# akofke/fountain

Measured on AMD Instinct MI355X. Metric: Mrays/s (primary+secondary) at fixed spp, higher is better.
Workload: dtype f32; 1 GPU; config 5 scene: 2309 baked copies of rounded_cube = 10002588 triangles (19979703 BVH nodes, depth 29), 4096x4096 film, PathIntegrator(max_depth 5, rr 1.0), 1024^2 env-map light; one step = 16 spp over the whole film; tiles=65536, tiles_per_gpu=65536, pipeline=wavefront, sampler=indexed xoshiro256+, per_gpu_workload=copies=2309,res=4096,spp_per_gpu=16

## Files before the change

fountain_amd/csrc/ftn_trace4.hip:

```cpp
#include "ftn_wf_common.h"

namespace ftn {

enum : uint32_t { T4_IDLE = 0, T4_NODE = 1, T4_LEAF = 2 };
#define T4_NONE 0xffffffffu

typedef float t4_f2 __attribute__((ext_vector_type(2)));
__device__ inline bool slab4(float4 a, float4 b, V3 o, V3 inv, float t_max, float* t0o, float* t1o) {
    const float k = 1.0f + 2.0f * gamma_n(3);
    const t4_f2 px = {a.x, a.y}, py = {a.z, a.w}, pz = {b.x, b.y};
    const t4_f2 tx = (px - (t4_f2){o.x, o.x}) * (t4_f2){inv.x, inv.x};
    const t4_f2 ty = (py - (t4_f2){o.y, o.y}) * (t4_f2){inv.y, inv.y};
    const t4_f2 tz = (pz - (t4_f2){o.z, o.z}) * (t4_f2){inv.z, inv.z};
    const float far_k = fmin_(fmin_(fmax_(tx.x, tx.y), fmax_(ty.x, ty.y)), fmax_(tz.x, tz.y)) * k;
    const float t0 = fmax_(fmax_(fmax_(0.0f, fmin_(tx.x, tx.y)), fmin_(ty.x, ty.y)), fmin_(tz.x, tz.y));
    const float t1 = fmin_(t_max, far_k);
    *t0o = t0; *t1o = t1;
    return !(t0 > t1);
}

struct WaveQueue {
    uint32_t chunk_next, chunk_end, slice, slices_done, chunk; bool exhausted;
};
__device__ inline void wq_init(WaveQueue& q, uint32_t count, uint32_t chunk_max) {
// ... 110 lines not shown
    const float4 q0 = rec[0], q1 = rec[1], q2 = rec[2], q3 = rec[3], q4 = rec[4], q5 = rec[5], q6 = rec[6], q7 = rec[7];
    float ta, tb, tc, td, x1;
    const bool ha = slab4(q0, q1, R.o, R.inv, R.t_max, &ta, &x1), hb = slab4(q2, q3, R.o, R.inv, R.t_max, &tb, &x1);
    const bool hc = slab4(q4, q5, R.o, R.inv, R.t_max, &tc, &x1), hd = slab4(q6, q7, R.o, R.inv, R.t_max, &td, &x1);
    const uint32_t ea = ha ? __float_as_uint(q1.z) : T4_NONE, eb = hb ? __float_as_uint(q3.z) : T4_NONE, ec = hc ? __float_as_uint(q5.z) : T4_NONE, ed = hd ? __float_as_uint(q7.z) : T4_NONE;
    t4_visit<CHECK>(St, L, R.t_max, ea, eb, ec, ed, ta, tb, tc, td, __float_as_uint(q1.w) & R.neg24);
}

template <bool CHECK>
__device__ __forceinline__ void t4q_record_step(const DScene& S, T4Stack<uint2>& St, T4Lane& L, V3 o, V3 inv, float t_max, uint32_t neg24) {
    const uint4* rec = reinterpret_cast<const uint4*>(reinterpret_cast<const char*>(S.quad64) + L.cur);
    const uint4 r0 = rec[0], r1 = rec[1], r2 = rec[2], r3 = rec[3];
    const float k2 = 1.0f + 4.0f * gamma_n(3);
    const T8Axis X = t8_axis(__uint_as_float(r0.x), r0.w & 0xffu, o.x, inv.x, r1.x, r1.x, r1.y, r1.y);
    const T8Axis Y = t8_axis(__uint_as_float(r0.y), (r0.w >> 8) & 0xffu, o.y, inv.y, r1.z, r1.z, r1.w, r1.w);
    const T8Axis Z = t8_axis(__uint_as_float(r0.z), (r0.w >> 16) & 0xffu, o.z, inv.z, r2.x, r2.x, r2.y, r2.y);
    float ta, a1, tb, b1, tc, c1, td, d1;
    T8_CHILD(0, ta, a1) T8_CHILD(1, tb, b1) T8_CHILD(2, tc, c1) T8_CHILD(3, td, d1)
    const uint32_t ea = !(ta > a1) ? r2.z : T4_NONE, eb = !(tb > b1) ? r2.w : T4_NONE, ec = !(tc > c1) ? r3.x : T4_NONE, ed = !(td > d1) ? r3.y : T4_NONE;
    t4_visit<CHECK>(St, L, t_max, ea, eb, ec, ed, ta, tb, tc, td, r3.z & neg24);
}

enum : uint32_t { T4_LEAF_IN = 3 };
template <bool COUNT, bool SPHERES, int BURST, bool Q64 = false>
__global__ void __launch_bounds__(256, (SPHERES ? 1 : (Q64 ? T4Q_WAVES : 5))) k_wf_trace4(DScene S, WfBuffers W, const uint32_t* __restrict__ queue, const uint32_t* count_ptr, uint32_t* head, DevStats* stats,
                                                   uint32_t refill, uint32_t leaf_batch, uint32_t chunk_max, uint32_t lds_entries, uint2* __restrict__ spill, uint32_t spill_levels) {
    T4Stack<uint2> St;
    extern __shared__ uint2 lds_stack2[];
    St.base = lds_stack2 + threadIdx.x;
    St.lim = St.base + 256u * lds_entries; St.sp = St.base; St.spill = spill; St.spill_levels = spill_levels;
    St.n_lanes = (size_t)gridDim.x * 256u; St.gl = (size_t)blockIdx.x * 256u + threadIdx.x;
    const bool st_tiny = lds_entries < 3u;
    uint2* const st_soft = st_tiny ? St.base : St.lim - 3 * 256;
    const uint32_t count = *count_ptr;
    const uint32_t lane = lane_id();
    unsigned long long n_rec = 0, n_prim = 0;
    unsigned long long occ[7] = {0, 0, 0, 0, 0, 0, 0};
    T4Lane L; L.mode = T4_IDLE; L.cur = 0; L.lp = 0; L.finish = false;
    WaveQueue Q; wq_init(Q, count, chunk_max);
    uint32_t rid = 0;
    RaySetup R; R.o = V3(0.0f, 0.0f, 0.0f); R.inv = R.o; R.dorig = R.o; R.t_max = 0.0f; R.neg24 = 0; R.kz = 0; R.sx = R.sy = R.sz = 0.0f;
    int hprim = -1; float hb0 = 0.0f, hb1 = 0.0f, hb2 = 0.0f; bool found = false;
    const float4 rlo = make_float4(S.root_lo[0], S.root_lo[1], S.root_lo[2], 0.0f), rhi = make_float4(S.root_hi[0], S.root_hi[1], S.root_hi[2], 0.0f);
    for (;;) {
        const unsigned long long idle = __ballot(L.mode == T4_IDLE);
        if (!Q.exhausted && (uint32_t)__popcll(idle) >= refill) {
            const uint32_t need = (uint32_t)__popcll(idle);
            if (wq_refill(Q, count, head, lane)) {
                if (W.drain_sig && lane == 0 && atomicAdd(&W.counters[CTR(WFC_DRY_WAVES)], 1u) + 1u == W.drain_at)
                    __hip_atomic_store(W.drain_sig, W.drain_seq, __ATOMIC_RELAXED, __HIP_MEMORY_SCOPE_SYSTEM);
            }
            const uint32_t avail = Q.chunk_end - Q.chunk_next;
            const uint32_t rank = (uint32_t)__popcll(idle & ((1ull << lane) - 1ull));
            bool hand_back = false; uint32_t q_entry = 0;
            if (COUNT) { occ[5]++; occ[6] += need < avail ? need : avail; }
            if (L.mode == T4_IDLE && rank < avail) {
                float4 a, b;
                q_entry = queue[Q.chunk_next + rank];
                load_queued_ray<false>(W, q_entry, &a, &b, &rid);
                ray_setup<SPHERES>(R, a, b);
                St.sp = St.base; L.cur = 0; found = false; hprim = -1; hb0 = 0.0f; hb1 = 0.0f; hb2 = 0.0f;
                if (ray_is_exceptional(R.o.x, R.o.y, R.o.z, R.inv.x, R.inv.y, R.inv.z) || (Q64 && ray_out_of_range8(R.o.x, R.o.y, R.o.z, R.inv.x, R.inv.y, R.inv.z)))
                    hand_back = true;
                else if (S.n_nodes == 0 || !slab_test(rlo, rhi, R.o, R.inv, R.t_max)) { W.hit[rid] = make_float4(FTN_INF, 0.0f, 0.0f, 0.0f); W.hit_prim[rid] = -1; }
                else if (S.root_is_leaf) { L.lp = 0; L.mode = T4_LEAF; }
                else L.mode = T4_NODE;
            }
            if (__ballot(hand_back) != 0) wave_push(hand_back, q_entry, W.q_exc_closest, &W.counters[CTR(WFC_EXC_CLOSEST)]);
            Q.chunk_next += (need < avail ? need : avail);
        }
        const unsigned long long m_node = __ballot(L.mode == T4_NODE), m_leaf = __ballot(L.mode >= T4_LEAF);
        if ((m_node | m_leaf) == 0) { if (Q.exhausted) break; else continue; }
        L.finish = false;
        if (COUNT) occ[0]++;
        if (m_node != 0 && (uint32_t)__popcll(m_leaf) < leaf_batch) {
#pragma unroll
            for (int burst = 0; burst < BURST; burst++) {
                const bool on = L.mode == T4_NODE && !L.finish;
                if (COUNT && on) n_rec++;
                if (COUNT) { const unsigned long long m_on = __ballot(on); if (m_on) { occ[1]++; occ[2] += (unsigned long long)__popcll(m_on); } }
                if (__builtin_expect(__ballot(on && (st_tiny || St.sp > st_soft)) == 0, 1)) {
                    if (on) { if (Q64) t4q_record_step<false>(S, St, L, R.o, R.inv, R.t_max, R.neg24); else t4_record_step<false>(S, R, St, L); }
// ... 306 lines not shown
        const uint32_t wg_q = knob_wg_closest ? knob_wg_closest : (uint32_t)T4Q_WAVES, budget_q = ((158u * 1024u) / wg_q) & ~1023u;
        const uint32_t bound_q = S.quad64_stack_bound ? S.quad64_stack_bound : 1u;
        uint32_t eq = knob_entries_closest ? knob_entries_closest : budget_q / (256u * 8u);
        p.entries_q64 = eq < bound_q ? eq : bound_q;
        if (p.entries_q64 == 0) p.entries_q64 = 1;
        p.spill_q64 = bound_q - p.entries_q64;
        p.lds_q64 = (size_t)p.entries_q64 * 256u * 8u;
        p.grid_q64 = (unsigned)n_cu * per_cu(p.lds_q64, wg_q);
        p.q64_ok = true;
    }
    if (S.oct && S.n_octs) {
        const uint32_t wg_8 = knob_wg_oct ? knob_wg_oct : 5u, budget_8 = ((158u * 1024u) / wg_8) & ~1023u, bound8 = S.oct_stack_bound ? S.oct_stack_bound : 1u;
        const uint32_t e8 = knob_entries_oct ? knob_entries_oct : budget_8 / (256u * 4u);
        p.entries_oct = e8 < bound8 ? e8 : bound8;
        p.spill_oct = bound8 - p.entries_oct;
        p.lds_oct = (size_t)p.entries_oct * 256u * 4u;
        p.grid_oct = (unsigned)n_cu * per_cu(p.lds_oct, wg_8);
        p.oct_ok = true;
    }
    return p;
}

void launch_trace4(int kind, bool count, bool spheres, unsigned grid, size_t lds, uint32_t lds_entries, void* spill, hipStream_t stream, const DScene& S, const WfBuffers& W,
                   const uint32_t* queue, const uint32_t* count_ptr, uint32_t* head, DevStats* stats, uint32_t refill, uint32_t leaf_batch, uint32_t chunk, uint32_t burst, uint32_t any_policy, uint32_t spill_levels) {
    const bool any = kind == T4K_ANY || kind == T4K_ANY_OCT;
#define FTN_T4(K, SPILL_T, ...) hipLaunchKernelGGL((K<__VA_ARGS__>), dim3(grid), dim3(256), lds, stream, S, W, queue, count_ptr, head, stats, refill, leaf_batch, chunk, lds_entries, (SPILL_T)spill, spill_levels)
    if (kind == T4K_CLOSEST_Q64) {
        if (count) FTN_T4(k_wf_trace4, uint2*, true, false, 2, true);
        else if (burst <= 1) FTN_T4(k_wf_trace4, uint2*, false, false, 1, true); else if (burst == 2) FTN_T4(k_wf_trace4, uint2*, false, false, 2, true);
        else if (burst == 3) FTN_T4(k_wf_trace4, uint2*, false, false, 3, true); else FTN_T4(k_wf_trace4, uint2*, false, false, 4, true);
    } else if (kind == T4K_ANY_OCT) {
#define FTN_T8(C, B) do { if (any_policy == 0) FTN_T4(k_wf_trace8_any, uint32_t*, C, B, 0); else FTN_T4(k_wf_trace8_any, uint32_t*, C, B, 1); } while (0)
        if (count) FTN_T8(true, 2);
        else if (burst <= 1) FTN_T8(false, 1); else if (burst == 2) FTN_T8(false, 2); else FTN_T8(false, 3);
#undef FTN_T8
    } else if (any) {
#define FTN_T4A(C, Sp, B) do { if (any_policy == 0) FTN_T4(k_wf_trace4_any, uint32_t*, C, Sp, B, 0); else FTN_T4(k_wf_trace4_any, uint32_t*, C, Sp, B, 1); } while (0)
        if (count) { if (spheres) FTN_T4A(true, true, 2); else FTN_T4A(true, false, 2); }
        else if (spheres) { if (burst <= 2) FTN_T4A(false, true, 2); else FTN_T4A(false, true, 4); }
        else { if (burst <= 1) FTN_T4A(false, false, 1); else if (burst == 2) FTN_T4A(false, false, 2); else if (burst == 3) FTN_T4A(false, false, 3); else FTN_T4A(false, false, 4); }
#undef FTN_T4A
    } else {
        if (count) { if (spheres) FTN_T4(k_wf_trace4, uint2*, true, true, 2); else FTN_T4(k_wf_trace4, uint2*, true, false, 2); }
        else if (spheres) { if (burst <= 2) FTN_T4(k_wf_trace4, uint2*, false, true, 2); else FTN_T4(k_wf_trace4, uint2*, false, true, 4); }
        else { if (burst <= 1) FTN_T4(k_wf_trace4, uint2*, false, false, 1); else if (burst == 2) FTN_T4(k_wf_trace4, uint2*, false, false, 2); else if (burst == 3) FTN_T4(k_wf_trace4, uint2*, false, false, 3); else FTN_T4(k_wf_trace4, uint2*, false, false, 4); }
    }
#undef FTN_T4
}

}
// ... 1 lines not shown
```

fountain_amd/csrc/ftn_wavefront.hip:

```cpp
#include "ftn_wf_internal.h"
#include "ftn_wf_path.h"
#include "ftn_texture.h"
#include <algorithm>
#include <cstdlib>
#include <cstring>
#include <vector>

namespace ftn {

__global__ void __launch_bounds__(256) k_wf_generate(RenderParams P, WfBuffers W, int write_state) {
    const uint32_t i = blockIdx.x * 256u + threadIdx.x;
    if (i >= W.n_paths) return;
    const uint32_t slot = i / W.samples, s = i % W.samples;
    const DTile tile = P.tiles[slot >> 8];
    const int px = tile.x0 + (int)(slot & 15u), py = tile.y0 + (int)((slot >> 4) & 15u);
    if (px < tile.x1 && py < tile.y1) {
        Rng rng; rng.seed(indexed_key(P.seed, px, py, W.first_sample + s));
        V2 j = rng.next2();
        V2 p_film((float)px + j.x, (float)py + j.y);
        V2 p_lens = rng.next2();
        float time_u = rng.next();
        DRay ray = camera_ray(P.C, p_film, p_lens, time_u);
        W.ray[2 * (size_t)(i)] = make_float4(ray.o.x, ray.o.y, ray.o.z, 0.0f);
        W.ray[2 * (size_t)(i) + 1] = make_float4(ray.d.x, ray.d.y, ray.d.z, ray.t_max);
        if (write_state) {
            W.beta[i] = make_float4(1.0f, 1.0f, 1.0f, __uint_as_float(PS_ALIVE));
            W.rad[i] = make_float4(0.0f, 0.0f, 0.0f, 0.0f);
            W.rng01[i] = make_ulonglong2(rng.s0, rng.s1); W.rng23[i] = make_ulonglong2(rng.s2, rng.s3);
        }
        uint32_t local = (uint32_t)(py - tile.y0) * (uint32_t)(tile.x1 - tile.x0) + (uint32_t)(px - tile.x0);
        if (W.gen_blocks && tile.x1 - tile.x0 == 16 && tile.y1 - tile.y0 == 16) {
            const uint32_t x = slot & 15u, y = (slot >> 4) & 15u;
            local = (x & 1u) | ((y & 1u) << 1) | ((x & 2u) << 1) | ((y & 2u) << 2) | ((x & 4u) << 2) | ((y & 4u) << 3) | ((x & 8u) << 3) | ((y & 8u) << 4);
        }
        const uint32_t pix = tile.valid_off + local;
        const uint32_t qi = pix * W.samples + s;
        W.q_active[0][qi] = i | (P.max_depth == 0 ? WF_Q_DEPTH : 0u);
        W.q_closest[qi] = i;
    }
}

__global__ void k_wf_reset(WfBuffers W, int mode, int in_q, DevStats* stats) {
    if (threadIdx.x != 0 || blockIdx.x != 0) return;
    if (mode == 0) {
        for (int i = 0; i < WFC_SLOTS; i++) W.counters[CTR(i)] = 0;
#ifdef FTN_DRAIN_PROBE
        for (int k = 0; k < 32; k++) W.counters[CTR(WFC_DRAIN_PROBE) + k] = 0;
#endif
        W.counters[CTR(WFC_ACTIVE_A)] = W.samples * W.valid_per_sample; W.counters[CTR(WFC_CLOSEST)] = W.samples * W.valid_per_sample;
        stats->camera_samples += (unsigned long long)W.samples * W.valid_per_sample;
    } else if (mode == 1) {
// ... 123 lines not shown
        uint32_t* const qs[2] = {W.q_active[out_q], W.q_closest};
        uint32_t* const cs[2] = {&W.counters[CTR(out_q == 0 ? WFC_ACTIVE_A : WFC_ACTIVE_B)], &W.counters[CTR(WFC_CLOSEST)]};
        block_push<2>(pred, val, qs, cs);
    }
    if (cam) atomicAdd(&P.stats->camera_samples, (unsigned long long)cam);
    if (spill) atomicAdd(&P.stats->spill_samples, (unsigned long long)spill);
    if (bc) atomicAdd(&P.stats->bc_writes, (unsigned long long)bc);
    if (err) atomicCAS(&P.stats->error, 0, err);
}

void launch_wf_new_pass(const WfBuffers& W, DevStats* stats, hipStream_t stream) { hipLaunchKernelGGL(k_wf_reset, dim3(1), dim3(64), 0, stream, W, 0, 0, stats); }
void launch_wf_generate(const RenderParams& P, const WfBuffers& W, int write_state, hipStream_t stream) {
    hipLaunchKernelGGL(k_wf_generate, dim3((W.n_paths + 255) / 256), dim3(256), 0, stream, P, W, write_state);
}

static int wavefront_render_serial(WavefrontState* st, const RenderParams& P, uint32_t n_tiles, bool count, bool count_production, hipStream_t stream, WavefrontTimes* times) {
    const bool tex = P.S.n_textures != 0;
    int rc = wf_reserve_serial(st, n_tiles, tex);
    if (rc) return rc;
    if ((rc = trace4_prepare(st, P.S))) return rc;
    WfBuffers W = st->W;
    W.serial = 1; W.ser_cursor = (uint2*)st->ser_mem[0]; W.ser_pfilm = (float2*)st->ser_mem[1]; W.ser_retired = (unsigned char*)st->ser_mem[2]; W.dfd = (float4*)st->ser_mem[3];
    W.n_slots = 0; W.samples = 1; W.n_paths = n_tiles; W.first_sample = 0; W.seg_cap = (uint32_t)st->cap_paths; W.valid_per_sample = 0;
    W.gen_blocks = 0; W.rng_replay = 0; W.br = nullptr; W.pd = nullptr; W.pd_md = 0; W.pd_occ = 0; W.late_finish = 0;
    const int count_mode = count ? (count_production ? 2 : 1) : 0;
    W.mis_any = ((!count || count_production) && knob("FTN_MIS_ANY", 1)) ? 1u : 0u;
    const bool spheres = P.S.n_spheres != 0;
    const size_t lds = wf_trace_lds(P.stack_entries);
    const unsigned tg = std::min<unsigned>(wf_trace_grid_max(st, lds), (2 * n_tiles + 255) / 256);
    const dim3 pgrid((n_tiles + 255) / 256);
    const unsigned sgrid = std::min<unsigned>((unsigned)st->n_cu * 8u, (n_tiles + 255) / 256);
    hipEvent_t e0 = st->ev[0], e1 = st->ev[1];
    (void)hipEventRecord(e0, stream);
    hipLaunchKernelGGL(k_wf_reset, dim3(1), dim3(64), 0, stream, W, 3, 0, P.stats);
    if (tex) hipLaunchKernelGGL((k_wf_serial_advance<true>), pgrid, dim3(256), 0, stream, P, W, 0, 1); else hipLaunchKernelGGL((k_wf_serial_advance<false>), pgrid, dim3(256), 0, stream, P, W, 0, 1);
    int in_q = 0; unsigned long long rounds = 0, trace_launches = 0;
    int polled_q[2] = {0, 0}; uint32_t* last = st->ser_host;
    const bool side_ok = st->side != nullptr && knob("FTN_WF_OVERLAP", 2) != 0 && getenv("ROCPROF_COUNTER_COLLECTION") == nullptr;
    const uint64_t max_rounds = 256u * (uint64_t)std::max<uint32_t>(P.spp, 1u) * ((uint64_t)P.max_depth + 4u + (1u << 12));
    for (uint64_t it = 0; it < max_rounds; it++) {
        const bool beside = it > 0 && side_ok;
        if (beside) { WF_TRY(hipEventRecord(st->ev_ready, stream)); WF_TRY(hipStreamWaitEvent(st->side, st->ev_ready, 0));
                      launch_trace(st, true, count_mode, spheres, tg, lds, st->side, P, W, W.q_shadow, &W.counters[CTR(WFC_SHADOW)], &W.counters[CTR(WFC_HEAD_ANY)], 2 * n_tiles);
                      WF_TRY(hipEventRecord(st->ev_side, st->side)); }
        launch_trace(st, false, count_mode, spheres, tg, lds, stream, P, W, W.q_closest, &W.counters[CTR(WFC_CLOSEST)], &W.counters[CTR(WFC_HEAD_CLOSEST)], 2 * n_tiles);
        trace_launches++;
        if (it > 0 && !beside) launch_trace(st, true, count_mode, spheres, tg, lds, stream, P, W, W.q_shadow, &W.counters[CTR(WFC_SHADOW)], &W.counters[CTR(WFC_HEAD_ANY)], 2 * n_tiles);
// ... 49 lines not shown
    const int count_mode = count ? (count_production ? 2 : 1) : 0;
    const bool dl_mode = P.integrator_kind != FTN_INTEGRATOR_PATH;
    const bool whitted = P.integrator_kind == FTN_INTEGRATOR_WHITTED;
    WfPassPlan plan;
    if ((rc = wf_plan_passes(st, P, tiles.size() * 256u, total_samples, dl_mode, &plan))) return rc;
    const uint32_t S = plan.samples;
    if ((rc = trace4_prepare(st, P.S))) return rc;
    if (dl_mode) { st->W.dlA = (float4*)st->dl_mem[0]; st->W.dlB = (float4*)st->dl_mem[1]; st->W.whT = (float4*)st->dl_mem[2]; st->W.dfd = (float4*)st->dl_mem[7]; }
    WfBuffers W = st->W;
    if (dl_mode) { W.sh = (float4*)st->dl_mem[3]; W.occluded = (unsigned char*)st->dl_mem[4]; W.q_shadow = (uint32_t*)st->dl_mem[5]; W.q_exc_any = (uint32_t*)st->dl_mem[6]; }
    if (!knob("FTN_ENV_CELLS_USE", 1)) P.S.env0.cells = nullptr;
    const bool spheres = P.S.n_spheres != 0;
    uint32_t valid = 0; for (const DTile& t : tiles) valid += (uint32_t)((t.x1 - t.x0) * (t.y1 - t.y0));
    W.valid_per_sample = valid;
    W.mis_any = ((!count || count_production) && knob("FTN_MIS_ANY", 1)) ? 1u : 0u;
    W.rng_replay = (!dl_mode && 5u + 8u * ((uint32_t)P.max_depth + 1u) <= 511u && knob("FTN_RNG_REPLAY", 1)) ? 1u : 0u;
    W.br = (!dl_mode && knob("FTN_WF_BR", 1)) ? st->br : nullptr;
    W.pd = (!dl_mode && knob("FTN_WF_PD", 3)) ? st->pd : nullptr;
    W.pd_md = (W.pd && knob("FTN_WF_PD", 3) >= 2) ? 1u : 0u;
    W.pd_occ = (W.pd && knob("FTN_WF_PD", 3) >= 3) ? 1u : 0u;
    W.gen_blocks = knob("FTN_GEN_BLOCKS", 1);
    W.late_finish = (!dl_mode && W.br && W.pd && W.pd_md && W.pd_occ && W.mis_any && P.S.env_only && knob("FTN_SHADE_ENV", 1) && knob("FTN_SHADE_SPECIALISE", 1) &&
                     knob("FTN_WF_LATE_FINISH", 1)) ? (hook ? 2u : 1u) : 0u;
    const size_t lds = wf_trace_lds(P.stack_entries);
    const unsigned trace_grid_max = wf_trace_grid_max(st, lds);
    const unsigned shade_grid_max = (unsigned)st->n_cu * 8u;
    double trace_ms = 0.0; unsigned long long trace_launches = 0, mis_any_rays = 0;
    double group_ms[4] = {0.0, 0.0, 0.0, 0.0}; unsigned long long group_n[4] = {0, 0, 0, 0};
    const uint32_t overlap_mode = knob("FTN_WF_OVERLAP", 2);
    const bool drain_gate = knob("FTN_WF_DRAIN_GATE", 1) != 0 && getenv("ROCPROF_COUNTER_COLLECTION") == nullptr;
    const uint32_t sort_bits = knob("FTN_WF_SORT", 0) ? std::min<uint32_t>(std::max<uint32_t>(knob("FTN_WF_SORT_BITS", 7), 1u), 9u) : 0u;
    uint32_t n_active = 0;
    int ev_used = 0;
    struct Span { int a, b, kind; };
    std::vector<Span> spans;
    static const char* const kGroup[4] = {"closest-hit trace", "any-hit trace", "classify + shade", "queue sort"};
    auto flush_events = [&]() -> int {
        if (spans.empty()) return FTN_OK;
        for (const Span& s : spans) WF_TRY(hipEventSynchronize(st->ev[s.b]));
        for (const Span& s : spans) {
            float ms = 0.0f; (void)hipEventElapsedTime(&ms, st->ev[s.a], st->ev[s.b]);
            group_ms[s.kind] += ms; group_n[s.kind]++;
            if (s.kind == 0) trace_ms += ms;
            if (knob("FTN_WF_DEBUG", 0)) fprintf(stderr, "[wf] %s: %.3f ms\n", kGroup[s.kind], ms);
        }
        spans.clear(); ev_used = 0;
        return FTN_OK;
    };
    auto span_begin = [&](hipStream_t sm) -> int { const int a = ev_used++; (void)hipEventRecord(st->ev[a], sm); return a; };
    auto span_end = [&](int a, int kind, hipStream_t sm) { const int b = ev_used++; (void)hipEventRecord(st->ev[b], sm); spans.push_back(Span{a, b, kind}); };
    auto render_passes = [&]() -> int {
    for (uint32_t s0 = 0; s0 < total_samples; s0 += S) {
        const uint32_t Sp = std::min(S, total_samples - s0);
        W.n_slots = n_slots; W.samples = Sp; W.n_paths = Sp * n_slots; W.first_sample = P.first_sample + s0; W.seg_cap = (uint32_t)st->cap_paths;
        hipLaunchKernelGGL(k_wf_reset, dim3(1), dim3(64), 0, stream, W, 0, 0, P.stats);
        hipLaunchKernelGGL(k_wf_generate, dim3((W.n_paths + 255) / 256), dim3(256), 0, stream, P, W, dl_mode ? 1 : 0);
        int in_q = 0;
        const uint32_t* q_cl = W.q_closest; const uint32_t* q_sh = W.q_shadow;
        const uint32_t max_iter = P.max_depth + 2 + (1u << 20);
        for (uint32_t it = 0; it < max_iter; it++) {
            bool polled = false;
            const unsigned tg = std::min<unsigned>(trace_grid_max, (2 * W.n_paths + 255) / 256);
            if (ev_used + 10 > 64) { rc = flush_events(); if (rc) return rc; }
#ifdef FTN_DRAIN_PROBE
            wf_set_probe_bounce(it);
#endif
            const bool overlap = overlap_mode == 1u || (overlap_mode == 2u && W.n_paths <= (32u << 20));
            const bool beside = overlap && it > 0 && q_sh == W.q_shadow;
            W.drain_sig = nullptr; W.drain_seq = 0;
            const bool gated = beside && st->drain_sig && drain_gate;
            if (beside) WF_TRY(hipEventRecord(st->ev_ready, stream));
            if (gated) {
                if (st->drain_seq >= 0xfffffff0u) { WF_TRY(hipStreamSynchronize(stream)); WF_TRY(hipStreamSynchronize(st->side)); WF_TRY(hipMemset(st->drain_sig, 0, 8)); st->drain_seq = 0; }
                W.drain_sig = st->drain_sig; W.drain_seq = ++st->drain_seq;
                W.drain_at = 1;
            }
            { const int e = span_begin(stream);
              launch_trace(st, false, count_mode, spheres, tg, lds, stream, P, W, q_cl, &W.counters[CTR(WFC_CLOSEST)], &W.counters[CTR(WFC_HEAD_CLOSEST)], 2 * W.n_paths,
                           it == 0 && W.samples >= knob("FTN_T4_LOCKSTEP_MIN_SPP", 1) );
              span_end(e, 0, stream); }
            if (gated) WF_TRY(hipStreamWriteValue32(stream, st->drain_sig, W.drain_seq, 0));
            trace_launches++;
            if (beside) WF_TRY(hipStreamWaitEvent(st->side, st->ev_ready, 0));
            if (gated) WF_TRY(hipStreamWaitValue32(st->side, st->drain_sig, W.drain_seq, hipStreamWaitValueGte, 0xffffffffu));
            if (it > 0) {
                const unsigned sg = std::min<unsigned>(trace_grid_max, (2 * W.n_paths + 255) / 256);
                hipStream_t as = beside ? st->side : stream;
                const int e = span_begin(as);
                launch_trace(st, true, count_mode, spheres, sg, lds, as, P, W, q_sh, &W.counters[CTR(WFC_SHADOW)], &W.counters[CTR(WFC_HEAD_ANY)], 2 * W.n_paths, it == 1 && W.samples >= 4u);
                span_end(e, 1, as);
                if (beside) WF_TRY(hipEventRecord(st->ev_side, st->side));
            }
            {
                const int e_cls = span_begin(stream);
                const unsigned cg = std::min<unsigned>(shade_grid_max, (W.n_paths + 255) / 256);
                hipLaunchKernelGGL(k_wf_reset, dim3(1), dim3(64), 0, stream, W, 2, in_q, P.stats);
                launch_wf_classify(P, W, in_q, (W.late_finish && it > 0) ? 0x3u : 0u, cg, stream);
                span_end(e_cls, 2, stream);
            }
            if (beside) WF_TRY(hipStreamWaitEvent(stream, st->ev_side, 0));
            const int e_shade = span_begin(stream);
            hipLaunchKernelGGL(k_wf_reset, dim3(1), dim3(64), 0, stream, W, 1, in_q, P.stats);
// ... 44 lines not shown
    if (rc) return rc;
    WF_TRY(hipGetLastError());
    if (times) {
        times->trace_ms = trace_ms; times->trace_launches = trace_launches; times->mis_any_rays = mis_any_rays;
        times->any_ms = group_ms[1]; times->any_launches = group_n[1]; times->shade_ms = group_ms[2]; times->shade_launches = group_n[2]; times->sort_ms = group_ms[3];
    }
    return FTN_OK;
}

#define WF_MAX_PASS_THROUGH 4096u
int wf_first_hit_passes(WavefrontState** state, const RenderParams& P, const std::vector<DTile>& tiles, const WfFirstHitPass& pass, hipStream_t stream, double* trace_ms_out) {
    knobs_begin();
    { int rc0 = wf_state_init(state); if (rc0) return rc0; }
    WavefrontState* st = *state;
    const uint32_t n_slots = (uint32_t)tiles.size() * 256u;
    const uint32_t total_samples = P.last_sample - P.first_sample;
    if (n_slots == 0 || total_samples == 0) return FTN_OK;
    WfPassPlan plan;
    int rc = wf_plan_passes(st, P, tiles.size() * 256u, total_samples, false, &plan);
    if (rc) return rc;
    const uint32_t S = plan.samples;
    if ((rc = trace4_prepare(st, P.S))) return rc;
    WfBuffers W = st->W;
    W.br = nullptr; W.pd = nullptr; W.pd_md = 0; W.pd_occ = 0; W.drain_sig = nullptr; W.drain_seq = 0; W.serial = 0; W.rng_replay = 0; W.mis_any = 0; W.late_finish = 0;
    W.gen_blocks = knob("FTN_GEN_BLOCKS", 1);
    uint32_t valid = 0; for (const DTile& t : tiles) valid += (uint32_t)((t.x1 - t.x0) * (t.y1 - t.y0));
    W.valid_per_sample = valid;
    if ((rc = pass.setup(st, valid))) return rc;
    const bool spheres = P.S.n_spheres != 0;
    const size_t lds = wf_trace_lds(P.stack_entries);
    const unsigned trace_grid_max = wf_trace_grid_max(st, lds);
    double trace_ms = 0.0;
    for (uint32_t s0 = 0; s0 < total_samples; s0 += S) {
        const uint32_t Sp = std::min(S, total_samples - s0);
        W.n_slots = n_slots; W.samples = Sp; W.n_paths = Sp * n_slots; W.first_sample = P.first_sample + s0; W.seg_cap = (uint32_t)st->cap_paths;
        launch_wf_new_pass(W, P.stats, stream);
        launch_wf_generate(P, W, 0, stream);
        const unsigned tg = std::min<unsigned>(trace_grid_max, (2 * W.n_paths + 255) / 256);
        uint32_t n_q = Sp * valid;
        for (uint32_t r = 0;; r++) {
            const bool odd = (r & 1u) != 0;
            const uint32_t* q_in = odd ? W.q_shadow : W.q_closest;
            uint32_t* q_out = odd ? W.q_closest : W.q_shadow;
            const uint32_t c_in = odd ? WFC_SHADOW : WFC_CLOSEST, c_out = odd ? WFC_CLOSEST : WFC_SHADOW;
            if (r > 0) hipLaunchKernelGGL(k_wf_round_reset, dim3(1), dim3(64), 0, stream, W, c_out);
            WF_TRY(hipEventRecord(st->ev[0], stream));
            launch_trace(st, false, 0, spheres, tg, lds, stream, P, W, q_in, &W.counters[CTR(c_in)], &W.counters[CTR(WFC_HEAD_CLOSEST)], 2 * W.n_paths,
// ... 22 lines not shown
```

fountain_amd/csrc/ftn_wf_common.h:

```cpp
#ifndef FTN_WF_COMMON_H
#define FTN_WF_COMMON_H
#include "ftn_wavefront.h"
#include "ftn_film.h"

namespace ftn {

enum : uint32_t { PS_BOUNCE_MASK = 0xffffu, PS_SPECULAR = 1u << 16, PS_ALIVE = 1u << 17, PS_DIRECT = 1u << 18, PS_SHADOW = 1u << 19, PS_MIS = 1u << 20, PS_DELTA = 1u << 21, PS_MIS_ANY = 1u << 22  };
#define PS_DRAWS_SHIFT 23
#define WF_MIS_BIT 0x80000000u

struct WfBuffers {
    uint32_t n_paths;
    uint32_t n_slots;
    uint32_t samples;
    uint32_t first_sample;
    float4 *ray;
    float4* hit;
    int* hit_prim;
    float4 *sh;
    unsigned char* occluded;
    float4 *beta;
    float4 *rad;
    float4* br;
    ulonglong2 *rng01, *rng23;
    float4 *pend0, *pend1, *pend2;
    float4* pd;
    uint32_t pd_md, pd_occ;
    uint32_t *q_active[2], *q_closest, *q_shadow;
    uint32_t* q_sorted;
    uint32_t* cls;
    uint32_t seg_cap;
    uint32_t* counters;
    uint32_t valid_per_sample;
    uint32_t* drain_sig; uint32_t drain_seq, drain_at;
    uint32_t *q_exc_closest, *q_exc_any;
    float4 *dlA, *dlB, *whT;
    float4* dfd;
    uint32_t serial;
    uint2* ser_cursor;
    float2* ser_pfilm;
    unsigned char* ser_retired;
    uint32_t rng_replay;
    uint32_t gen_blocks;
    uint32_t mis_any;
    uint32_t late_finish;
};

#define WF_Q_FIN 0x80000000u
#define WF_Q_DEPTH 0x40000000u
#define WF_Q_ID_MASK 0x0fffffffu

#define CTR(i) ((i) * 32)
enum : int {
    WFC_ACTIVE_A = 0, WFC_ACTIVE_B = 1,
    WFC_CLOSEST = 2, WFC_SHADOW = 3,
    WFC_NODE_STEPS = 6, WFC_LEAF_STEPS = 7, WFC_IDLE_LANES = 8, WFC_LEAFWAIT_LANES = 9,
    WFC_MIS_ANY = 10,
    WFC_DRY_WAVES = 11,
    WFC_DRAIN_PROBE = 13,
    WFC_HEADS_FIRST = 16,
    WFC_HEAD_CLOSEST = 16, WFC_HEAD_ANY = 24,
    WFC_HEADS_END = 32,
    WFC_EXC_FIRST = 32,
    WFC_EXC_CLOSEST = 32, WFC_EXC_ANY = 33, WFC_EXC_HEAD_CLOSEST = 40, WFC_EXC_HEAD_ANY = 48,
    WFC_EXC_END = 56,
    WFC_SLOTS = 64
};
#define WF_NCLASS 8
// ... 101 lines not shown
                if (hh && (fl & GF_HAS_UVS) && tri_uv_degenerate_reject(S, (int)prim, V3(g0.x, g0.y, g0.z), V3(g1.x, g1.y, g1.z), V3(g2.x, g2.y, g2.z))) hh = false;
            }
        }
    }
    *t_out = t; *b0o = b0; *b1o = b1; *b2o = b2;
    return hh;
}


struct Trace4Plan {
    uint32_t entries_closest, entries_any;
    uint32_t spill_closest, spill_any;
    size_t lds_closest, lds_any;
    unsigned grid_closest, grid_any;
    bool oct_ok; uint32_t entries_oct, spill_oct; size_t lds_oct; unsigned grid_oct;
    bool q64_ok; uint32_t entries_q64, spill_q64; size_t lds_q64; unsigned grid_q64;
};
enum : int { T4K_CLOSEST = 0, T4K_ANY = 1, T4K_ANY_OCT = 2, T4K_CLOSEST_Q64 = 3 };
#ifndef T4Q_WAVES
#define T4Q_WAVES 6
#endif
Trace4Plan trace4_plan(const DScene& S, int n_cu, uint32_t knob_entries_closest, uint32_t knob_entries_any, uint32_t knob_wg_closest, uint32_t knob_wg_any, uint32_t knob_wg_oct, uint32_t knob_entries_oct);
void launch_trace4(int kind, bool count, bool spheres, unsigned grid, size_t lds, uint32_t lds_entries, void* spill, hipStream_t stream, const DScene& S, const WfBuffers& W,
                   const uint32_t* queue, const uint32_t* count_ptr, uint32_t* head, DevStats* stats, uint32_t refill, uint32_t leaf_batch, uint32_t chunk, uint32_t burst, uint32_t any_policy, uint32_t spill_levels);

}
#endif
```

fountain_amd/csrc/ftn_wf_path.h:

```cpp
#ifndef FTN_WF_PATH_H
#define FTN_WF_PATH_H
#include "ftn_wf_common.h"

namespace ftn {

__device__ inline Rgb wf_add_direct(Rgb L, bool shadow_lit, float4 q0, float4 q1, float4 q2, Rgb inc, uint32_t n_lights) {
    Rgb radiance(0.0f);
    if (shadow_lit) radiance = radiance + Rgb(q0.x, q0.y, q0.z);
    if (!inc.is_black()) radiance = radiance + Rgb(q1.x, q1.y, q1.z) * inc * q0.w / q1.w;
    Rgb direct = Rgb(q2.x, q2.y, q2.z) * ((float)n_lights * radiance);
    return L + direct;
}
__device__ inline Rgb wf_add_seen(Rgb L, Rgb beta, Rgb e) { return L + beta * e; }
template <bool ENV> __device__ inline Rgb wf_escaped_Le(const DScene& S, V3 d) { return ENV ? Rgb(0.0f) + light_Le_env(S.env0, d) : scene_env_Le(S, d); }
__device__ inline Rgb wf_finish_path(const DScene& S, Rgb beta, Rgb L, uint32_t ps, float4 q0, float4 q1, float4 q2, float4 q3, bool hit, V3 d) {
    if (ps & PS_DIRECT) {
        const uint32_t occ_word = __float_as_uint(q3.w);
        Rgb inc(0.0f);
        if ((ps & PS_MIS_ANY) && !((occ_word & 0xff00u) != 0u)) inc = light_Le_env(S.env0, V3(q3.x, q3.y, q3.z));
        L = wf_add_direct(L, (ps & PS_SHADOW) && !((occ_word & 0xffu) != 0u), q0, q1, q2, inc, S.n_lights);
    }
    if ((ps & PS_ALIVE) && ((ps & PS_BOUNCE_MASK) == 0u || (ps & PS_SPECULAR) != 0u)) L = wf_add_seen(L, beta, hit ? Rgb(0.0f) : wf_escaped_Le<true>(S, d));
    return L;
}

}
#endif
// ... 1 lines not shown
```

fountain_amd/csrc/ftn_wf_state.cpp:

```cpp
#include "ftn_wf_internal.h"
#include <algorithm>
#include <cstdlib>
#include <string>
#include <unordered_map>

namespace ftn {

static thread_local std::string g_wf_err;
const char* wavefront_error() { return g_wf_err.c_str(); }
void wf_set_error(const std::string& msg) { g_wf_err = msg; }

int wf_grow(void** p, size_t* bytes, size_t need) {
    if (need <= *bytes) return FTN_OK;
    if (*p) (void)hipFree(*p);
    *p = nullptr; *bytes = 0;
    WF_TRY(hipMalloc(p, need));
    *bytes = need;
    return FTN_OK;
}

size_t wf_trace_lds(uint32_t stack_entries) { return (size_t)stack_entries * 256 * sizeof(uint32_t); }
unsigned wf_trace_grid_max(const WavefrontState* st, size_t lds) {
    const unsigned blocks_per_cu = (unsigned)std::max<size_t>(1, std::min<size_t>(8, (size_t)(160 * 1024) / std::max<size_t>(lds, 1)));
    return (unsigned)st->n_cu * blocks_per_cu;
// ... 10 lines not shown
    if (st->side) (void)hipStreamDestroy(st->side);
    if (st->drain_sig) (void)hipFree(st->drain_sig);
    for (void* m : st->dl_mem) if (m) (void)hipFree(m);
    for (void* m : st->ser_mem) if (m) (void)hipFree(m);
    if (st->t4_spill_c) (void)hipFree(st->t4_spill_c);
    if (st->t4_spill_a) (void)hipFree(st->t4_spill_a);
    if (st->host_counters) (void)hipHostFree(st->host_counters);
    if (st->ser_host) (void)hipHostFree(st->ser_host);
    delete st;
}
template <class T> static int wf_alloc(WavefrontState* st, T** p, size_t n) {
    WF_TRY(hipMalloc((void**)p, n * sizeof(T)));
    st->mem[st->n_mem++] = (void*)*p;
    return FTN_OK;
}
int wf_reserve(WavefrontState* st, size_t n) {
    if (n <= st->cap_paths) return FTN_OK;
    wf_free(st);
    WfBuffers& W = st->W; int rc;
    if ((rc = wf_alloc(st, &W.ray, 4 * n)) || (rc = wf_alloc(st, &W.hit, 2 * n)) || (rc = wf_alloc(st, &W.hit_prim, 2 * n)) ||
        (rc = wf_alloc(st, &W.sh, 2 * n)) || (rc = wf_alloc(st, &W.occluded, 2 * n)) || (rc = wf_alloc(st, &W.beta, n)) || (rc = wf_alloc(st, &W.rad, n)) ||
        (rc = wf_alloc(st, &W.rng01, n)) || (rc = wf_alloc(st, &W.rng23, n)) || (rc = wf_alloc(st, &W.pend0, n)) || (rc = wf_alloc(st, &W.pend1, n)) || (rc = wf_alloc(st, &W.pend2, n)) ||
        (rc = wf_alloc(st, &W.q_active[0], n)) || (rc = wf_alloc(st, &W.q_active[1], n)) || (rc = wf_alloc(st, &W.q_closest, 2 * n)) || (rc = wf_alloc(st, &W.q_shadow, 2 * n)) || (rc = wf_alloc(st, &W.q_sorted, 8 * n)) || (rc = wf_alloc(st, &W.cls, CTR(WF_NCLASS))) ||
        (rc = wf_alloc(st, &W.q_exc_closest, 2 * n)) || (rc = wf_alloc(st, &W.q_exc_any, 2 * n)) || (rc = wf_alloc(st, &W.counters, CTR(WFC_SLOTS))) || (rc = wf_alloc(st, &st->br, 2 * n)) || (rc = wf_alloc(st, &st->pd, 4 * n))) return rc;
    st->cap_paths = n;
    return FTN_OK;
}

static thread_local std::unordered_map<std::string, std::pair<bool, uint32_t>> g_knobs;
void knobs_begin() { g_knobs.clear(); }
uint32_t knob(const char* name, uint32_t def) {
    auto it = g_knobs.find(name);
    if (it == g_knobs.end()) { const char* v = getenv(name); it = g_knobs.emplace(name, std::make_pair(v != nullptr, v ? (uint32_t)atoi(v) : 0u)).first; }
    return it->second.first ? it->second.second : def;
}

void wf_free_dl(WavefrontState* st) { for (void*& m : st->dl_mem) { if (m) (void)hipFree(m); m = nullptr; } st->dl_paths = 0; st->dl_levels = 0; st->dl_slots = 0; st->dl_tex = false; }
int wf_reserve_dl(WavefrontState* st, size_t n, uint32_t levels, uint32_t slots, bool tex) {
    if (n <= st->dl_paths && levels <= st->dl_levels && slots <= st->dl_slots && (!tex || st->dl_tex)) return FTN_OK;
    wf_free_dl(st);
    const size_t sl = std::max<uint32_t>(slots, 2u);
    WF_TRY(hipMalloc(&st->dl_mem[0], (size_t)levels * n * sizeof(float4)));
    WF_TRY(hipMalloc(&st->dl_mem[1], (size_t)levels * n * sizeof(float4)));
    WF_TRY(hipMalloc(&st->dl_mem[2], (size_t)slots * n * sizeof(float4)));
    WF_TRY(hipMalloc(&st->dl_mem[3], 2 * (size_t)slots * n * sizeof(float4)));
    WF_TRY(hipMalloc(&st->dl_mem[4], sl * n));
    WF_TRY(hipMalloc(&st->dl_mem[5], sl * n * sizeof(uint32_t)));
// ... 84 lines not shown
```

fountain_amd/csrc/ftn_wf_trace.hip:

```cpp
#include "ftn_wf_internal.h"
#include <algorithm>
#include <cstring>
#include <string>
#include <hipcub/hipcub.hpp>

namespace ftn {

enum : uint32_t { TM_IDLE = 0, TM_NODE = 1, TM_LEAF = 2 };

template <bool ANY, bool COUNT, bool SPHERES, int BURST >
__global__ void __launch_bounds__(256) k_wf_trace(DScene S, WfBuffers W, const uint32_t* __restrict__ queue, const uint32_t* count_ptr, uint32_t* head,
                                                  DevStats* stats, uint32_t refill, uint32_t leaf_batch, uint32_t chunk, uint32_t node_burst) {
    extern __shared__ uint32_t lds_stack[];
    uint32_t* const st_base = lds_stack + threadIdx.x;
    uint32_t* sptr = st_base;
    const uint32_t count = *count_ptr;
    const uint32_t lane = lane_id();
    const uint32_t np = W.n_paths;
    TravCount tc{0, 0};
    uint32_t w_idle_lanes = 0, w_leafwait_lanes = 0;
    uint32_t w_node_steps = 0, w_leaf_steps = 0;
    uint32_t mode = TM_IDLE;
    uint32_t chunk_next = 0, chunk_end = 0; bool exhausted = count == 0;
    uint32_t slice = blockIdx.x & 7u, slices_done = 0;
// ... 254 lines not shown
    st->t8_on = st->t4.oct_ok && S.n_spheres == 0 && knob("FTN_T8", 1) != 0;
    const size_t need_a8 = st->t8_on ? (size_t)st->t4.grid_oct * 256u * st->t4.spill_oct * sizeof(uint32_t) : 0;
    const size_t need_a = std::max<size_t>(need_a8, (size_t)st->t4.grid_any * 256u * st->t4.spill_any * sizeof(uint32_t));
    int rc = wf_grow(&st->t4_spill_c, &st->t4_spill_c_bytes, need_c);
    if (!rc) rc = wf_grow(&st->t4_spill_a, &st->t4_spill_a_bytes, need_a);
    return rc;
}

void launch_trace(WavefrontState* st, bool any, int count, bool spheres, unsigned grid, size_t lds, hipStream_t stream, const RenderParams& P, const WfBuffers& W,
                  const uint32_t* queue, const uint32_t* count_ptr, uint32_t* head, uint32_t max_rays, bool camera_rays) {
    if (st->t4_on && count != 1) {
        const Trace4Plan& T = st->t4;
        const bool oct = any && st->t8_on, q64 = !any && st->q64_on;
        const unsigned g = std::min<unsigned>(oct ? T.grid_oct : (any ? T.grid_any : (q64 ? T.grid_q64 : T.grid_closest)), std::max<unsigned>(1u, (max_rays + 255u) / 256u));
        uint32_t chunk4 = knob("FTN_TRACE_CHUNK", 128);
        while (chunk4 > 64u && (uint64_t)chunk4 * g * 4u * 4u > (uint64_t)max_rays) chunk4 >>= 1;
        if (oct) launch_trace4(T4K_ANY_OCT, count == 2, false, g, T.lds_oct, T.entries_oct, st->t4_spill_a, stream, P.S, W, queue, count_ptr, head, P.stats,
                               camera_rays ? knob("FTN_T8_REFILL1", 16) : knob("FTN_T8_REFILL", 24), camera_rays ? knob("FTN_T8_LEAF_BATCH1", 16) : knob("FTN_T8_LEAF_BATCH", 16), chunk4, knob("FTN_T8_BURST", 2), knob("FTN_T8_POLICY", 1), T.spill_oct);
        else launch_trace4(any ? T4K_ANY : (q64 ? T4K_CLOSEST_Q64 : T4K_CLOSEST), count == 2, spheres, g, any ? T.lds_any : (q64 ? T.lds_q64 : T.lds_closest),
                      any ? T.entries_any : (q64 ? T.entries_q64 : T.entries_closest), any ? st->t4_spill_a : st->t4_spill_c, stream, P.S, W,
                      queue, count_ptr, head, P.stats,
                      any ? knob("FTN_T4_ANY_REFILL", 32) : (camera_rays ? knob("FTN_T4_REFILL0", 64) : knob("FTN_T4_REFILL", 32)),
                      any ? knob("FTN_T4_ANY_LEAF_BATCH", 16) : (camera_rays ? knob("FTN_T4_LEAF_BATCH0", 2) : knob("FTN_T4_LEAF_BATCH", 16)), chunk4,
                      any ? knob("FTN_T4_ANY_BURST", 4) : (camera_rays ? knob("FTN_T4_BURST0", 3) : knob("FTN_T4_BURST", 2)), knob("FTN_T4_ANY_POLICY", 1), any ? T.spill_any : (q64 ? T.spill_q64 : T.spill_closest));
        const unsigned ge = std::min<unsigned>(grid, (unsigned)st->n_cu);
        uint32_t* ecount = &W.counters[CTR(any ? WFC_EXC_ANY : WFC_EXC_CLOSEST)]; uint32_t* ehead = &W.counters[CTR(any ? WFC_EXC_HEAD_ANY : WFC_EXC_HEAD_CLOSEST)];
        DevStats* none = nullptr;
#define FTN_TRE(A, Sp) hipLaunchKernelGGL((k_wf_trace<A, false, Sp, 8>), dim3(ge), dim3(256), lds, stream, P.S, W, any ? W.q_exc_any : W.q_exc_closest, ecount, ehead, none, 24u, 2u, 64u, 8u)
        if (any) { if (spheres) FTN_TRE(true, true); else FTN_TRE(true, false); } else { if (spheres) FTN_TRE(false, true); else FTN_TRE(false, false); }
#undef FTN_TRE
        return;
    }
    const bool count_b = count != 0;
    const uint32_t refill = knob("FTN_TRACE_REFILL", 24), leaf_batch = knob("FTN_TRACE_LEAF_BATCH", 2), chunk_knob = knob("FTN_TRACE_CHUNK", 128), node_burst = knob("FTN_TRACE_BURST", 8);
    uint32_t chunk = chunk_knob;
    const uint32_t waves = grid * 4u;
    while (chunk > 64u && (uint64_t)chunk * waves * 4u > (uint64_t)max_rays) chunk >>= 1;
    if (any && !count_b && knob("FTN_TRACE_ANY2", 1) && P.S.fat) {
        const uint32_t refill2 = knob("FTN_ANY2_REFILL", 16), leaf_batch2 = knob("FTN_ANY2_LEAF_BATCH", leaf_batch);
        uint32_t policy2 = knob("FTN_ANY2_POLICY", 2);
#ifdef FTN_DRAIN_PROBE
        policy2 |= g_probe_bounce << 8;
#endif
        if (spheres) hipLaunchKernelGGL((k_wf_trace_any2<true>), dim3(grid), dim3(256), lds, stream, P.S, W, queue, count_ptr, head, P.stats, refill2, leaf_batch2, chunk, policy2);
        else hipLaunchKernelGGL((k_wf_trace_any2<false>), dim3(grid), dim3(256), lds, stream, P.S, W, queue, count_ptr, head, P.stats, refill2, leaf_batch2, chunk, policy2);
        return;
    }
// ... 54 lines not shown
```

Measured before the change: 3337 Mrays/s.

## Generate camera rays inside the first trace kernel instead of the generate pass

```diff
diff --git a/fountain_amd/csrc/ftn_trace4.hip b/fountain_amd/csrc/ftn_trace4.hip
--- a/fountain_amd/csrc/ftn_trace4.hip
+++ b/fountain_amd/csrc/ftn_trace4.hip
@@ -1,4 +1,4 @@
-#include "ftn_wf_common.h"
+#include "ftn_wf_path.h"
 
 namespace ftn {
 
@@ -156,7 +156,22 @@
 }
 
 enum : uint32_t { T4_LEAF_IN = 3 };
-template <bool COUNT, bool SPHERES, int BURST, bool Q64 = false>
+struct T4RayRecord { float4 a, b; };
+__device__ __noinline__ T4RayRecord t4_camera_ray(const WfCamKey* cam, uint32_t samples, uint32_t first_sample, uint32_t p) {
+    const __attribute__((address_space(4))) WfCamKey* K = (const __attribute__((address_space(4))) WfCamKey*)cam;
+    DCamera C;
+#pragma unroll
+    for (int i = 0; i < 16; i++) { C.c2w[i] = K->C.c2w[i]; C.r2c[i] = K->C.r2c[i]; }
+    C.shutter_open = K->C.shutter_open; C.shutter_close = K->C.shutter_close; C.lens_radius = K->C.lens_radius; C.focal_dist = K->C.focal_dist;
+#pragma unroll
+    for (int i = 0; i < 3; i++) { C.dx_camera[i] = K->C.dx_camera[i]; C.dy_camera[i] = K->C.dy_camera[i]; }
+    const uint32_t slot = p / samples, s = p - slot * samples;
+    Rng rng;
+    const DRay r = wf_camera_ray(C, K->seed, K->tiles[slot >> 8], slot, first_sample + s, &rng);
+    T4RayRecord rec; rec.a = make_float4(r.o.x, r.o.y, r.o.z, 0.0f); rec.b = make_float4(r.d.x, r.d.y, r.d.z, r.t_max);
+    return rec;
+}
+template <bool COUNT, bool SPHERES, int BURST, bool Q64 = false, bool CAM = false>
 __global__ void __launch_bounds__(256, (SPHERES ? 1 : (Q64 ? T4Q_WAVES : 5))) k_wf_trace4(DScene S, WfBuffers W, const uint32_t* __restrict__ queue, const uint32_t* count_ptr, uint32_t* head, DevStats* stats,
                                                    uint32_t refill, uint32_t leaf_batch, uint32_t chunk_max, uint32_t lds_entries, uint2* __restrict__ spill, uint32_t spill_levels) {
     T4Stack<uint2> St;
@@ -191,7 +206,11 @@
             if (L.mode == T4_IDLE && rank < avail) {
                 float4 a, b;
                 q_entry = queue[Q.chunk_next + rank];
-                load_queued_ray<false>(W, q_entry, &a, &b, &rid);
+                if (CAM) {
+                    rid = q_entry; const T4RayRecord rec = t4_camera_ray(W.cam, W.samples, W.first_sample, rid); a = rec.a; b = rec.b;
+                    W.ray[2 * (size_t)rid] = a; W.ray[2 * (size_t)rid + 1] = b;
+                }
+                else load_queued_ray<false>(W, q_entry, &a, &b, &rid);
                 ray_setup<SPHERES>(R, a, b);
                 St.sp = St.base; L.cur = 0; found = false; hprim = -1; hb0 = 0.0f; hb1 = 0.0f; hb2 = 0.0f;
                 if (ray_is_exceptional(R.o.x, R.o.y, R.o.z, R.inv.x, R.inv.y, R.inv.z) || (Q64 && ray_out_of_range8(R.o.x, R.o.y, R.o.z, R.inv.x, R.inv.y, R.inv.z)))
@@ -544,10 +563,14 @@
 }
 
 void launch_trace4(int kind, bool count, bool spheres, unsigned grid, size_t lds, uint32_t lds_entries, void* spill, hipStream_t stream, const DScene& S, const WfBuffers& W,
-                   const uint32_t* queue, const uint32_t* count_ptr, uint32_t* head, DevStats* stats, uint32_t refill, uint32_t leaf_batch, uint32_t chunk, uint32_t burst, uint32_t any_policy, uint32_t spill_levels) {
+                   const uint32_t* queue, const uint32_t* count_ptr, uint32_t* head, DevStats* stats, uint32_t refill, uint32_t leaf_batch, uint32_t chunk, uint32_t burst, uint32_t any_policy, uint32_t spill_levels, bool cam_key) {
     const bool any = kind == T4K_ANY || kind == T4K_ANY_OCT;
 #define FTN_T4(K, SPILL_T, ...) hipLaunchKernelGGL((K<__VA_ARGS__>), dim3(grid), dim3(256), lds, stream, S, W, queue, count_ptr, head, stats, refill, leaf_batch, chunk, lds_entries, (SPILL_T)spill, spill_levels)
-    if (kind == T4K_CLOSEST_Q64) {
+    if (kind == T4K_CLOSEST_Q64 && cam_key) {
+        if (count) FTN_T4(k_wf_trace4, uint2*, true, false, 2, true, true);
+        else if (burst <= 1) FTN_T4(k_wf_trace4, uint2*, false, false, 1, true, true); else if (burst == 2) FTN_T4(k_wf_trace4, uint2*, false, false, 2, true, true);
+        else if (burst == 3) FTN_T4(k_wf_trace4, uint2*, false, false, 3, true, true); else FTN_T4(k_wf_trace4, uint2*, false, false, 4, true, true);
+    } else if (kind == T4K_CLOSEST_Q64) {
         if (count) FTN_T4(k_wf_trace4, uint2*, true, false, 2, true);
         else if (burst <= 1) FTN_T4(k_wf_trace4, uint2*, false, false, 1, true); else if (burst == 2) FTN_T4(k_wf_trace4, uint2*, false, false, 2, true);
         else if (burst == 3) FTN_T4(k_wf_trace4, uint2*, false, false, 3, true); else FTN_T4(k_wf_trace4, uint2*, false, false, 4, true);
diff --git a/fountain_amd/csrc/ftn_wavefront.hip b/fountain_amd/csrc/ftn_wavefront.hip
--- a/fountain_amd/csrc/ftn_wavefront.hip
+++ b/fountain_amd/csrc/ftn_wavefront.hip
@@ -10,23 +10,22 @@
 
 __global__ void __launch_bounds__(256) k_wf_generate(RenderParams P, WfBuffers W, int write_state) {
     const uint32_t i = blockIdx.x * 256u + threadIdx.x;
+    if (i == 0 && W.cam_key) { W.cam->C = P.C; W.cam->seed = P.seed; W.cam->tiles = P.tiles; }
     if (i >= W.n_paths) return;
     const uint32_t slot = i / W.samples, s = i % W.samples;
     const DTile tile = P.tiles[slot >> 8];
     const int px = tile.x0 + (int)(slot & 15u), py = tile.y0 + (int)((slot >> 4) & 15u);
     if (px < tile.x1 && py < tile.y1) {
-        Rng rng; rng.seed(indexed_key(P.seed, px, py, W.first_sample + s));
-        V2 j = rng.next2();
-        V2 p_film((float)px + j.x, (float)py + j.y);
-        V2 p_lens = rng.next2();
-        float time_u = rng.next();
-        DRay ray = camera_ray(P.C, p_film, p_lens, time_u);
-        W.ray[2 * (size_t)(i)] = make_float4(ray.o.x, ray.o.y, ray.o.z, 0.0f);
-        W.ray[2 * (size_t)(i) + 1] = make_float4(ray.d.x, ray.d.y, ray.d.z, ray.t_max);
-        if (write_state) {
-            W.beta[i] = make_float4(1.0f, 1.0f, 1.0f, __uint_as_float(PS_ALIVE));
-            W.rad[i] = make_float4(0.0f, 0.0f, 0.0f, 0.0f);
-            W.rng01[i] = make_ulonglong2(rng.s0, rng.s1); W.rng23[i] = make_ulonglong2(rng.s2, rng.s3);
+        if (!W.cam_key) {
+            Rng rng;
+            const DRay ray = wf_camera_ray(P.C, P.seed, tile, slot, W.first_sample + s, &rng);
+            W.ray[2 * (size_t)(i)] = make_float4(ray.o.x, ray.o.y, ray.o.z, 0.0f);
+            W.ray[2 * (size_t)(i) + 1] = make_float4(ray.d.x, ray.d.y, ray.d.z, ray.t_max);
+            if (write_state) {
+                W.beta[i] = make_float4(1.0f, 1.0f, 1.0f, __uint_as_float(PS_ALIVE));
+                W.rad[i] = make_float4(0.0f, 0.0f, 0.0f, 0.0f);
+                W.rng01[i] = make_ulonglong2(rng.s0, rng.s1); W.rng23[i] = make_ulonglong2(rng.s2, rng.s3);
+            }
         }
         uint32_t local = (uint32_t)(py - tile.y0) * (uint32_t)(tile.x1 - tile.x0) + (uint32_t)(px - tile.x0);
         if (W.gen_blocks && tile.x1 - tile.x0 == 16 && tile.y1 - tile.y0 == 16) {
@@ -196,7 +195,7 @@
     WfBuffers W = st->W;
     W.serial = 1; W.ser_cursor = (uint2*)st->ser_mem[0]; W.ser_pfilm = (float2*)st->ser_mem[1]; W.ser_retired = (unsigned char*)st->ser_mem[2]; W.dfd = (float4*)st->ser_mem[3];
     W.n_slots = 0; W.samples = 1; W.n_paths = n_tiles; W.first_sample = 0; W.seg_cap = (uint32_t)st->cap_paths; W.valid_per_sample = 0;
-    W.gen_blocks = 0; W.rng_replay = 0; W.br = nullptr; W.pd = nullptr; W.pd_md = 0; W.pd_occ = 0; W.late_finish = 0;
+    W.gen_blocks = 0; W.rng_replay = 0; W.br = nullptr; W.pd = nullptr; W.pd_md = 0; W.pd_occ = 0; W.late_finish = 0; W.cam_key = 0;
     const int count_mode = count ? (count_production ? 2 : 1) : 0;
     W.mis_any = ((!count || count_production) && knob("FTN_MIS_ANY", 1)) ? 1u : 0u;
     const bool spheres = P.S.n_spheres != 0;
@@ -292,6 +291,7 @@
     W.gen_blocks = knob("FTN_GEN_BLOCKS", 1);
     W.late_finish = (!dl_mode && W.br && W.pd && W.pd_md && W.pd_occ && W.mis_any && P.S.env_only && knob("FTN_SHADE_ENV", 1) && knob("FTN_SHADE_SPECIALISE", 1) &&
                      knob("FTN_WF_LATE_FINISH", 1)) ? (hook ? 2u : 1u) : 0u;
+    const bool cam_key_ok = !dl_mode && hook == nullptr && st->t4_on && st->q64_on && count_mode != 1 && knob("FTN_WF_CAM_KEY", 1) != 0;
     const size_t lds = wf_trace_lds(P.stack_entries);
     const unsigned trace_grid_max = wf_trace_grid_max(st, lds);
     const unsigned shade_grid_max = (unsigned)st->n_cu * 8u;
@@ -323,6 +323,8 @@
     for (uint32_t s0 = 0; s0 < total_samples; s0 += S) {
         const uint32_t Sp = std::min(S, total_samples - s0);
         W.n_slots = n_slots; W.samples = Sp; W.n_paths = Sp * n_slots; W.first_sample = P.first_sample + s0; W.seg_cap = (uint32_t)st->cap_paths;
+        const bool camera_launch = Sp >= knob("FTN_T4_LOCKSTEP_MIN_SPP", 1);
+        W.cam_key = (cam_key_ok && camera_launch) ? 1u : 0u;
         hipLaunchKernelGGL(k_wf_reset, dim3(1), dim3(64), 0, stream, W, 0, 0, P.stats);
         hipLaunchKernelGGL(k_wf_generate, dim3((W.n_paths + 255) / 256), dim3(256), 0, stream, P, W, dl_mode ? 1 : 0);
         int in_q = 0;
@@ -347,7 +349,7 @@
             }
             { const int e = span_begin(stream);
               launch_trace(st, false, count_mode, spheres, tg, lds, stream, P, W, q_cl, &W.counters[CTR(WFC_CLOSEST)], &W.counters[CTR(WFC_HEAD_CLOSEST)], 2 * W.n_paths,
-                           it == 0 && W.samples >= knob("FTN_T4_LOCKSTEP_MIN_SPP", 1) );
+                           it == 0 && camera_launch);
               span_end(e, 0, stream); }
             if (gated) WF_TRY(hipStreamWriteValue32(stream, st->drain_sig, W.drain_seq, 0));
             trace_launches++;
@@ -438,7 +440,7 @@
     const uint32_t S = plan.samples;
     if ((rc = trace4_prepare(st, P.S))) return rc;
     WfBuffers W = st->W;
-    W.br = nullptr; W.pd = nullptr; W.pd_md = 0; W.pd_occ = 0; W.drain_sig = nullptr; W.drain_seq = 0; W.serial = 0; W.rng_replay = 0; W.mis_any = 0; W.late_finish = 0;
+    W.br = nullptr; W.pd = nullptr; W.pd_md = 0; W.pd_occ = 0; W.drain_sig = nullptr; W.drain_seq = 0; W.serial = 0; W.rng_replay = 0; W.mis_any = 0; W.late_finish = 0; W.cam_key = 0;
     W.gen_blocks = knob("FTN_GEN_BLOCKS", 1);
     uint32_t valid = 0; for (const DTile& t : tiles) valid += (uint32_t)((t.x1 - t.x0) * (t.y1 - t.y0));
     W.valid_per_sample = valid;
diff --git a/fountain_amd/csrc/ftn_wf_common.h b/fountain_amd/csrc/ftn_wf_common.h
--- a/fountain_amd/csrc/ftn_wf_common.h
+++ b/fountain_amd/csrc/ftn_wf_common.h
@@ -8,6 +8,8 @@
 enum : uint32_t { PS_BOUNCE_MASK = 0xffffu, PS_SPECULAR = 1u << 16, PS_ALIVE = 1u << 17, PS_DIRECT = 1u << 18, PS_SHADOW = 1u << 19, PS_MIS = 1u << 20, PS_DELTA = 1u << 21, PS_MIS_ANY = 1u << 22  };
 #define PS_DRAWS_SHIFT 23
 #define WF_MIS_BIT 0x80000000u
+
+struct WfCamKey { DCamera C; unsigned long long seed; const DTile* tiles; };
 
 struct WfBuffers {
     uint32_t n_paths;
@@ -44,6 +46,8 @@
     uint32_t gen_blocks;
     uint32_t mis_any;
     uint32_t late_finish;
+    uint32_t cam_key;
+    WfCamKey* cam;
 };
 
 #define WF_Q_FIN 0x80000000u
@@ -191,7 +195,8 @@
 #endif
 Trace4Plan trace4_plan(const DScene& S, int n_cu, uint32_t knob_entries_closest, uint32_t knob_entries_any, uint32_t knob_wg_closest, uint32_t knob_wg_any, uint32_t knob_wg_oct, uint32_t knob_entries_oct);
 void launch_trace4(int kind, bool count, bool spheres, unsigned grid, size_t lds, uint32_t lds_entries, void* spill, hipStream_t stream, const DScene& S, const WfBuffers& W,
-                   const uint32_t* queue, const uint32_t* count_ptr, uint32_t* head, DevStats* stats, uint32_t refill, uint32_t leaf_batch, uint32_t chunk, uint32_t burst, uint32_t any_policy, uint32_t spill_levels);
+                   const uint32_t* queue, const uint32_t* count_ptr, uint32_t* head, DevStats* stats, uint32_t refill, uint32_t leaf_batch, uint32_t chunk, uint32_t burst, uint32_t any_policy, uint32_t spill_levels,
+                   bool cam_key = false );
 
 }
 #endif
diff --git a/fountain_amd/csrc/ftn_wf_path.h b/fountain_amd/csrc/ftn_wf_path.h
--- a/fountain_amd/csrc/ftn_wf_path.h
+++ b/fountain_amd/csrc/ftn_wf_path.h
@@ -3,6 +3,16 @@
 #include "ftn_wf_common.h"
 
 namespace ftn {
+
+__device__ inline DRay wf_camera_ray(DCamera C, unsigned long long seed, DTile tile, uint32_t slot, uint32_t sample, Rng* rng) {
+    const int px = tile.x0 + (int)(slot & 15u), py = tile.y0 + (int)((slot >> 4) & 15u);
+    rng->seed(indexed_key(seed, px, py, sample));
+    const V2 j = rng->next2();
+    const V2 p_film((float)px + j.x, (float)py + j.y);
+    const V2 p_lens = rng->next2();
+    const float time_u = rng->next();
+    return camera_ray(C, p_film, p_lens, time_u);
+}
 
 __device__ inline Rgb wf_add_direct(Rgb L, bool shadow_lit, float4 q0, float4 q1, float4 q2, Rgb inc, uint32_t n_lights) {
     Rgb radiance(0.0f);
diff --git a/fountain_amd/csrc/ftn_wf_state.cpp b/fountain_amd/csrc/ftn_wf_state.cpp
--- a/fountain_amd/csrc/ftn_wf_state.cpp
+++ b/fountain_amd/csrc/ftn_wf_state.cpp
@@ -56,7 +56,8 @@
         (rc = wf_alloc(st, &W.sh, 2 * n)) || (rc = wf_alloc(st, &W.occluded, 2 * n)) || (rc = wf_alloc(st, &W.beta, n)) || (rc = wf_alloc(st, &W.rad, n)) ||
         (rc = wf_alloc(st, &W.rng01, n)) || (rc = wf_alloc(st, &W.rng23, n)) || (rc = wf_alloc(st, &W.pend0, n)) || (rc = wf_alloc(st, &W.pend1, n)) || (rc = wf_alloc(st, &W.pend2, n)) ||
         (rc = wf_alloc(st, &W.q_active[0], n)) || (rc = wf_alloc(st, &W.q_active[1], n)) || (rc = wf_alloc(st, &W.q_closest, 2 * n)) || (rc = wf_alloc(st, &W.q_shadow, 2 * n)) || (rc = wf_alloc(st, &W.q_sorted, 8 * n)) || (rc = wf_alloc(st, &W.cls, CTR(WF_NCLASS))) ||
-        (rc = wf_alloc(st, &W.q_exc_closest, 2 * n)) || (rc = wf_alloc(st, &W.q_exc_any, 2 * n)) || (rc = wf_alloc(st, &W.counters, CTR(WFC_SLOTS))) || (rc = wf_alloc(st, &st->br, 2 * n)) || (rc = wf_alloc(st, &st->pd, 4 * n))) return rc;
+        (rc = wf_alloc(st, &W.q_exc_closest, 2 * n)) || (rc = wf_alloc(st, &W.q_exc_any, 2 * n)) || (rc = wf_alloc(st, &W.counters, CTR(WFC_SLOTS))) || (rc = wf_alloc(st, &st->br, 2 * n)) || (rc = wf_alloc(st, &st->pd, 4 * n)) ||
+        (rc = wf_alloc(st, &W.cam, 1))) return rc;
     st->cap_paths = n;
     return FTN_OK;
 }
diff --git a/fountain_amd/csrc/ftn_wf_trace.hip b/fountain_amd/csrc/ftn_wf_trace.hip
--- a/fountain_amd/csrc/ftn_wf_trace.hip
+++ b/fountain_amd/csrc/ftn_wf_trace.hip
@@ -300,7 +300,8 @@
                       queue, count_ptr, head, P.stats,
                       any ? knob("FTN_T4_ANY_REFILL", 32) : (camera_rays ? knob("FTN_T4_REFILL0", 64) : knob("FTN_T4_REFILL", 32)),
                       any ? knob("FTN_T4_ANY_LEAF_BATCH", 16) : (camera_rays ? knob("FTN_T4_LEAF_BATCH0", 2) : knob("FTN_T4_LEAF_BATCH", 16)), chunk4,
-                      any ? knob("FTN_T4_ANY_BURST", 4) : (camera_rays ? knob("FTN_T4_BURST0", 3) : knob("FTN_T4_BURST", 2)), knob("FTN_T4_ANY_POLICY", 1), any ? T.spill_any : (q64 ? T.spill_q64 : T.spill_closest));
+                      any ? knob("FTN_T4_ANY_BURST", 4) : (camera_rays ? knob("FTN_T4_BURST0", 3) : knob("FTN_T4_BURST", 2)), knob("FTN_T4_ANY_POLICY", 1), any ? T.spill_any : (q64 ? T.spill_q64 : T.spill_closest),
+                      q64 && camera_rays && W.cam_key != 0);
         const unsigned ge = std::min<unsigned>(grid, (unsigned)st->n_cu);
         uint32_t* ecount = &W.counters[CTR(any ? WFC_EXC_ANY : WFC_EXC_CLOSEST)]; uint32_t* ehead = &W.counters[CTR(any ? WFC_EXC_HEAD_ANY : WFC_EXC_HEAD_CLOSEST)];
         DevStats* none = nullptr;
```

Result: no change. 3347 Mrays/s (median of 6 runs) (+0.3%).
